# gcorso/disco-diffdock

Measured on AMD Instinct MI355X. Metric: complexes/sec, 20-step 40-sample inference, higher is better.
Workload: dtype f32

## Files before the change

disco_diffdock_amd/csrc/ddk_capi.hip:

```cpp
#include <math.h>
#include <algorithm>
#include <cmath>
#include <string.h>

#include "model.h"
#include "k_conv_common.h"

using namespace ddk;

namespace ddk {


int fail(ddk_ctx* ctx, int code, const std::string& msg) {
  if (ctx) ctx->err = msg;
  return code;
}

int hip_fail(ddk_ctx* ctx, hipError_t e, const char* what) {
  return fail(ctx, DDK_ERR_HIP, std::string(what) + ": " + hipGetErrorString(e));
}

hipError_t ctx_malloc(ddk_ctx* ctx, void** p, size_t bytes) {
  *p = nullptr;
  if (ctx->alloc_limit > 0 && ctx->dev_bytes + (int64_t)bytes > ctx->alloc_limit) { ctx->alloc_refusals++; return hipErrorOutOfMemory; }
// ... 306 lines not shown
  if (!bw || !bb || !bm || !bv) return DDK_ERR_INVALID;
  int ch = 0, f = 0;
  const int dims[4] = {1, 3, 3, 1};
  for (int b = 0; b < 4; ++b)
    for (int m = 0; m < out[b]; ++m, ++f) {
      const float sc = powf(bv->data[f] + 1e-5f, -0.5f) * bw->data[f];
      for (int d = 0; d < dims[b]; ++d, ++ch) {
        scale[ch] = sc;
        if (b == 0) { mean[ch] = bm->data[m]; bias[ch] = bb->data[m]; }
      }
    }
  return DDK_OK;
}

static int pack_x3(ddk_ctx* ctx, ConvLayerDev& L, int NG, const std::vector<float>& w1all, const std::vector<float>& w2all,
                   const std::vector<float>& b2all) {
  const size_t w1sz = 3 * 9 * 64 * 4, w2sz = (size_t)L.n_tiles * 9 * 64 * 4, b2sz = (size_t)L.n_tiles * 32;
  const int limbs = ctx->cfg.conv_kernel == 3 ? 3 : 2;
  const int tile_bytes = limbs == 3 ? W2X_TILE_BYTES : W2X2_TILE_BYTES, bias_off = limbs == 3 ? W2X_BIAS_OFF : W2X2_BIAS_OFF,
            desc_off = limbs == 3 ? W2X_DESC_OFF : W2X2_DESC_OFF, w1_tile_bytes = limbs == 3 ? W1X_TILE_BYTES : W1X2_TILE_BYTES;
  bool exact = true;
  auto split = [&exact, limbs](float v, uint16_t& hi, uint16_t& mid, uint16_t& lo) {
    const _Float16 h = (_Float16)v;
    const float r1 = v - (float)h;
    const _Float16 m = (_Float16)r1;
    const _Float16 l = (_Float16)(r1 - (float)m);
    memcpy(&hi, &h, 2); memcpy(&mid, &m, 2); memcpy(&lo, &l, 2);
    if (limbs == 3) {
      const double back = (double)(float)h + (double)(float)m + (double)(float)l;
      if (std::fabs(v) >= 0.5f ? back != (double)v : std::fabs(back - (double)v) > 0x1p-25) exact = false;
    } else {
      const double back = (double)(float)h + (double)(float)m;
      if (std::fabs(back - (double)v) > std::max(0x1p-22 * std::fabs((double)v), 0x1p-25)) exact = false;
    }
  };
  auto range_scale = [](const float* v, size_t n, const float* v2, size_t n2) {
    float m = 0.f;
    for (size_t i = 0; i < n; ++i) m = std::max(m, std::fabs(v[i]));
    for (size_t i = 0; i < n2; ++i) m = std::max(m, std::fabs(v2[i]));
    int e = 0;
    std::frexp(std::max(m, 0x1p-40f), &e);
    return std::ldexp(1.0f, 15 - e);
  };
  std::vector<uint8_t> w2x((size_t)(NG * L.n_tiles + 4) * tile_bytes, 0), w1x((size_t)NG * 3 * w1_tile_bytes, 0);
  auto frags = [&](const float* src, float sc, uint8_t* dst) {
    for (int r = 0; r < 36; ++r)
      for (int lane = 0; lane < 64; ++lane) {
        const float v = src[((size_t)(r / 4) * 64 + lane) * 4 + (r & 3)] * sc;
        const int s_ = r / 8, i = r % 8;
        const size_t off = s_ < 4 ? (size_t)s_ * 1024 + lane * 16 + 2 * i : (size_t)4096 + lane * 8 + 2 * i;
        uint16_t h, m, l;
        split(v, h, m, l);
        memcpy(dst + off, &h, 2); memcpy(dst + W2X_LIMB_BYTES + off, &m, 2);
        if (limbs == 3) memcpy(dst + 2 * W2X_LIMB_BYTES + off, &l, 2);
      }
  };
  for (int g = 0; g < NG; ++g) {
    const float* w2 = w2all.data() + g * w2sz;
    const float* w1 = w1all.data() + g * w1sz;
    const float* b2 = b2all.data() + g * b2sz;
    const float sc1 = range_scale(w1, w1sz, nullptr, 0), sc2 = range_scale(w2, w2sz, nullptr, 0);
    L.w1s[g] = sc1; L.w2s[g] = sc2;
    for (int t = 0; t < L.n_tiles; ++t) {
      uint8_t* rec = w2x.data() + ((size_t)g * L.n_tiles + t) * tile_bytes;
      frags(w2 + (size_t)t * 2304, sc2, rec);
      memcpy(rec + bias_off, b2 + (size_t)t * 32, 128);
      const int32_t dq[2] = {x_tile_word(L.h_tiles[t].w0), L.h_tiles[t].chan0};
      if (dq[0] < 0) return fail(ctx, DDK_ERR_INVALID, "internal: a vector tile of the conv layout does not sit on a T1O / T1E row quad");
      memcpy(rec + desc_off, dq, 8);
    }
    for (int T = 0; T < 3; ++T) frags(w1 + (size_t)T * 2304, sc1, w1x.data() + ((size_t)g * 3 + T) * w1_tile_bytes);
  }
  if (!exact)
    return fail(ctx, DDK_ERR_INVALID, limbs == 3 ? "internal: the three-limb fp16 split of a conv weight is not exact"
                                                 : "internal: the two-limb fp16 split of a conv weight leaves its 2^-22 window");
  L.h_w2x = w2x; L.h_w1x = w1x;
  L.epi_ok = conv_epilogue_shapes_ok(L.h_tiles);
  L.limbs = limbs;
  if (ctx->host_only) return DDK_OK;
  L.w2x = (uint8_t*)dev_alloc(ctx, w2x.size());
  L.w1x = (uint8_t*)dev_alloc(ctx, w1x.size());
  if (!L.w2x || !L.w1x) return fail(ctx, DDK_ERR_NOMEM, "device allocation failed while packing conv weights (f16 limbs)");
  if (hipMemcpy(L.w2x, w2x.data(), w2x.size(), hipMemcpyHostToDevice) != hipSuccess ||
      hipMemcpy(L.w1x, w1x.data(), w1x.size(), hipMemcpyHostToDevice) != hipSuccess)
    return fail(ctx, DDK_ERR_HIP, "f16-limb weight upload failed");
  return DDK_OK;
}

static int build_conv_layer(ddk_ctx* ctx, int mode, int l, ConvLayerDev& L) {
  const ddk_config& c = ctx->cfg;
  const int ns = c.ns;
  std::vector<int> rowmap;
  std::vector<float> rowscale;
  std::vector<TileDesc> tiles;
  int rc = build_layout(ctx, mode, l, L, rowmap, rowscale, tiles);
  if (rc) return rc;
  const int NG = mode == 0 ? 4 : 9;
// ... 69 lines not shown
  L.h_bn_bias.assign((size_t)n_bn * XW, 0.f);
  if (c.batch_norm)
    for (int g = 0; g < n_bn; ++g) {
      const std::string pre = "conv_layers." + std::to_string(mode == 0 ? l : 9 * l + g) + ".batch_norm";
      if ((rc = fold_batch_norm(ctx, pre, L.out_mul, L.h_bn_mean.data() + (size_t)g * XW, L.h_bn_scale.data() + (size_t)g * XW,
                                L.h_bn_bias.data() + (size_t)g * XW)))
        return rc;
    }
  L.h_w1p.resize(NG); L.h_b1p.resize(NG); L.h_w2p.resize(NG); L.h_b2p.resize(NG);
  for (int g = 0; g < NG; ++g) {
    L.h_w1p[g].assign(w1all.begin() + g * w1sz, w1all.begin() + (g + 1) * w1sz);
    L.h_b1p[g].assign(b1all.begin() + g * b1sz, b1all.begin() + (g + 1) * b1sz);
    L.h_w2p[g].assign(w2all.begin() + g * w2sz, w2all.begin() + (g + 1) * w2sz);
    L.h_b2p[g].assign(b2all.begin() + g * b2sz, b2all.begin() + (g + 1) * b2sz);
  }
  if (mode == 0 && c.conv_kernel != 1 && (rc = pack_x3(ctx, L, NG, w1all, w2all, b2all))) return rc;
  if (mode == 1 && c.conv_kernel != 1) {
    std::vector<int> rmx = rowmap;
    std::vector<float> rsx = rowscale;
    for (int t = 0; t + 1 < L.n_tiles; ++t) {
      if ((tiles[t].w0 & 3) != T_TV || (tiles[t].w0 >> 16) != F_T2E) continue;
      if ((tiles[t + 1].w0 & 3) != T_TV || (tiles[t + 1].w0 >> 16) != F_T2E + 12) return fail(ctx, DDK_ERR_INVALID, "internal: the two tiles of a T2E row group are not adjacent");
      for (int rq = 0; rq < 3; ++rq)
        for (int hh = 0; hh < 2; ++hh) {
          const size_t a = (size_t)t * 32 + 8 * rq + 4 * hh, b = (size_t)(t + 1) * 32 + 8 * rq + 4 * hh;
          if (rowmap[b + 2] >= 0 || rowmap[b + 3] >= 0) return fail(ctx, DDK_ERR_INVALID, "internal: a T2E row group holds more than six rows");
          for (int j = 0; j < 2; ++j) {
            rmx[a + j] = -1; rsx[a + j] = 0.f;
            rmx[a + 2 + j] = rowmap[a + j]; rsx[a + 2 + j] = rowscale[a + j];
            rmx[b + j] = rowmap[a + 2 + j]; rsx[b + j] = rowscale[a + 2 + j];
            rmx[b + 2 + j] = rowmap[b + j]; rsx[b + 2 + j] = rowscale[b + j];
// ... 363 lines not shown
    ConvLayerDev& L = head ? ctx->head[l - 100] : ctx->conv[l];
    if (g < 0 || g >= L.n_groups) return fail(ctx, DDK_ERR_INVALID, "bad export index");
    const std::string it(item);
    if (it == "w1p") { src = L.h_w1p[g].data(); n = L.h_w1p[g].size(); }
    else if (it == "b1p") { src = L.h_b1p[g].data(); n = L.h_b1p[g].size(); }
    else if (it == "w2p") { src = L.h_w2p[g].data(); n = L.h_w2p[g].size(); }
    else if (it == "b2p") { src = L.h_b2p[g].data(); n = L.h_b2p[g].size(); }
    else if (it == "wn") { src = L.h_wn.data(); n = L.h_wn.size(); }
    else if (it == "bnp") { src = L.h_bnp.data(); n = L.h_bnp.size(); }
    else if (it == "tiles") { src = L.h_tiles.data(); n = L.h_tiles.size() * (sizeof(TileDesc) / 4); }
    else if (it == "bn_mean") { src = L.h_bn_mean.data(); n = L.h_bn_mean.size(); }
    else if (it == "bn_scale") { src = L.h_bn_scale.data(); n = L.h_bn_scale.size(); }
    else if (it == "bn_bias") { src = L.h_bn_bias.data(); n = L.h_bn_bias.size(); }
    else if (it == "w1x") { src = L.h_w1x.data(); n = L.h_w1x.size() / 4; }
    else if (it == "w2x") { src = L.h_w2x.data(); n = L.h_w2x.size() / 4; }
    else if (it == "xscale") { static thread_local float sc[8]; for (int k = 0; k < 4; ++k) { sc[k] = L.w1s[k]; sc[4 + k] = L.w2s[k]; } src = sc; n = 8; }
    else return fail(ctx, DDK_ERR_INVALID, "unknown export item");
  } else {
    return fail(ctx, DDK_ERR_INVALID, "unknown export name");
  }
  if (buf) {
    if (cap_words < n) return fail(ctx, DDK_ERR_INVALID, "export buffer too small");
    memcpy(buf, src, (size_t)n * 4);
  }
  return n;
}

int ddk_debug_split3(ddk_ctx* ctx, const float* x, int64_t n, int32_t group, float* hi, float* mid, float* lo, float* scale, void* stream) {
  if (!ctx || ctx->host_only) return DDK_ERR_STATE;
  if (n < 0 || group < 1 || !x || !hi || !mid || !lo || !scale) return fail(ctx, DDK_ERR_INVALID, "ddk_debug_split3: bad argument");
// ... 6 lines not shown
```

disco_diffdock_amd/csrc/ddk_internal.h:

```cpp
#pragma once
#include <hip/hip_runtime.h>
#include <stdint.h>

#include <map>
#include <string>
#include <vector>

#include "../../include/ddk.h"
#include "../../include/ddk_debug.h"

namespace ddk {

constexpr int NS = 24;
constexpr int NV = 6;
constexpr int XW = 2 * NS + 6 * NV;
constexpr int NE = 3 * NS;
constexpr int OFF_P = NS;
constexpr int OFF_Q = NS + 3 * NV;
constexpr int OFF_C = NS + 6 * NV;

constexpr int F_A = 0;
constexpr int F_C = NS;
constexpr int F_T1O = 2 * NS;
constexpr int F_T1E = F_T1O + 6 * NV;
// ... 15 lines not shown
template <int MODE> struct ConvTraits;
template <> struct ConvTraits<0> { static constexpr int WAVES = CONV_WAVES, FS = F_STRIDE; };
template <> struct ConvTraits<1> { static constexpr int WAVES = 6, FS = F_STRIDE2; };
template <int MODE> constexpr size_t conv_lds_bytes() { return (size_t)(ConvTraits<MODE>::WAVES * 32 * ConvTraits<MODE>::FS + 2 * W2_TILE_FLOATS + 16) * 4; }
static_assert(conv_lds_bytes<1>() <= 160 * 1024, "LDS budget (l<=2)");
constexpr int CONV_MAX_GROUPS = 9;
constexpr int W2X_LIMB_BYTES = 4 * 1024 + 512;
constexpr int W2X_BIAS_OFF = 3 * W2X_LIMB_BYTES;
constexpr int W2X_DESC_OFF = W2X_BIAS_OFF + 128;
constexpr int W2X_TILE_BYTES = W2X_DESC_OFF + 16;
constexpr int W1X_TILE_BYTES = 3 * W2X_LIMB_BYTES;
constexpr int W2X2_BIAS_OFF = 2 * W2X_LIMB_BYTES;
constexpr int W2X2_DESC_OFF = W2X2_BIAS_OFF + 128;
constexpr int W2X2_TILE_BYTES = W2X2_DESC_OFF + 16;
constexpr int W1X2_TILE_BYTES = 2 * W2X_LIMB_BYTES;
constexpr int W1L_LIMB_BYTES = 1024 + 512;
constexpr int W1L_BYTES = 3 * 2 * W1L_LIMB_BYTES;
constexpr int CONV_TRACE_TILES = 1024;
constexpr int FX_A = 0, FX_C = NS, FX_R = 2 * NS, FX_PQ = FX_R + 6 * NV, FX_STRIDE = FX_PQ + 12 + 4;
static_assert(FX_STRIDE == 100 && FX_A == F_A && FX_C == F_C, "F row layout (three-limb f16)");
constexpr int W2X_STAGES = 4;
constexpr size_t CONV_X_LDS_BYTES = (size_t)CONV_WAVES * 32 * FX_STRIDE * 4 + W2X_STAGES * W2X_TILE_BYTES + 16;
static_assert(CONV_X_LDS_BYTES <= 160 * 1024 && W2X_TILE_BYTES % 16 == 0, "LDS budget (three-limb f16)");
constexpr size_t CONV_X2_LDS_BYTES = (size_t)CONV_WAVES * 32 * FX_STRIDE * 4 + W2X_STAGES * W2X2_TILE_BYTES + W1L_BYTES + 16;
static_assert(CONV_X2_LDS_BYTES <= 160 * 1024 && W2X2_TILE_BYTES % 16 == 0 && W1L_BYTES % 16 == 0, "LDS budget (two-limb f16)");

enum TileKind : int {
  T_RA = 0,
  T_RT = 1,
  T_TV = 2,
  T_RTS = 3
};
// ... 32 lines not shown
      if (first != odd) w0 |= 0x4000 << half;
    }
  }
  return (w0 & 0xffff) | (nf << 16);
}

struct ConvLayerDev {
  int n_tiles = 0;
  bool has_weights = false;
  int W = 0;
  int din = 0, dout = 0;
  float* w1p[4] = {};
  float* b1p[4] = {};
  float* w2r[4] = {};
  uint8_t* w1x = nullptr;
  uint8_t* w2x = nullptr;
  float w1s[CONV_MAX_GROUPS] = {1, 1, 1, 1, 1, 1, 1, 1, 1}, w2s[CONV_MAX_GROUPS] = {1, 1, 1, 1, 1, 1, 1, 1, 1};
  int limbs = 2;
  bool epi_ok = false;
  int n_cols = 0;
  int col_start[17] = {};
  float* wn = nullptr;
  float* bnp = nullptr;
  std::vector<float> h_wn, h_bnp;
  float* bn_mean = nullptr;
  float* bn_scale = nullptr;
  float* bn_bias = nullptr;
  std::vector<std::vector<float>> h_w1p, h_b1p, h_w2p, h_b2p;
  std::vector<float> h_bn_mean, h_bn_scale, h_bn_bias;
  int n_groups = 4;
  std::vector<TileDesc> h_tiles;
  std::vector<uint8_t> h_w1x, h_w2x;
  int n_in[4] = {}, n_out[4] = {}, blk_off[4] = {};
  int in_mul[4] = {}, out_mul[4] = {};
};

constexpr int PRE_W = 4 * NE;
static inline int pre_pos(int o) {
  const int r32 = o < 64 ? o % 32 : o - 64, hh = (r32 >> 2) & 1;
  return o < 64 ? hh * 36 + (o / 32) * 16 + (r32 & 3) + 4 * (r32 >> 3) : hh * 36 + 32 + (r32 & 3);
}

struct HostTensor {
  std::vector<int64_t> shape;
  std::vector<float> data;
};

// ... 116 lines not shown
```

disco_diffdock_amd/csrc/k_conv.hip:

```cpp
#include <stdlib.h>

#include "k_conv_common.h"
#include "k_node.h"
#include "model.h"

namespace ddk {

__device__ __forceinline__ void load_frags(float4 (&a)[9], f32x16& B, const float* w, const float* b) {
#pragma unroll
  for (int s4 = 0; s4 < 9; ++s4) a[s4] = ld4(w + s4 * 256);
#pragma unroll
  for (int j = 0; j < 4; ++j) {
    const float4 v = ld4(b + 4 * j);
    B[4 * j + 0] = v.x; B[4 * j + 1] = v.y; B[4 * j + 2] = v.z; B[4 * j + 3] = v.w;
  }
}

__device__ __forceinline__ f32x16 burst(const float4 (&a)[9], const float (&h)[36], const f32x16& C) {
  f32x16 D = MFMA(a[0].x, h[0], C);
  D = MFMA(a[0].y, h[1], D);
  D = MFMA(a[0].z, h[2], D);
  D = MFMA(a[0].w, h[3], D);
#pragma unroll
  for (int s4 = 1; s4 < 9; ++s4) {
// ... 486 lines not shown
  float* row = (A.sum_g2 != nullptr && g == 2) ? A.sum_g2 + (size_t)(s_last - A.g2_node_off) * XW
                                               : A.sum + ((size_t)s_last * A.n_slots + ((A.slots >> (2 * g)) & 3)) * XW;
  if (lane < dout) row[lane] = acc0;
  if (lane + 64 < dout) row[lane + 64] = acc1;
}

void conv_det_fix(const ConvKArgs& k, const ConvLaunch& a, int dout, hipStream_t s) {
  const int64_t tiles = a.edge_bound / 32 + 8 * CONV_MAX_GROUPS + (int64_t)CONV_WAVES * a.det_nr;
  hipLaunchKernelGGL(conv_det_fix_kernel, dim3((unsigned)((tiles + 3) / 4)), dim3(256), 0, s, k, dout);
}

hipError_t launch_conv_fused(const ConvLayerDev& L, const ConvLaunch& a, int n_cu, hipStream_t s) {
  if (L.w2x != nullptr && (a.mode == 0 || (a.mode == 1 && a.pre == nullptr)))
    return L.limbs == 2 ? launch_conv_fused_x2(L, a, n_cu, s) : launch_conv_fused_x(L, a, n_cu, s);
  ConvKArgs k;
  k.w1x = nullptr; k.w2x = nullptr;
  for (int g = 0; g < CONV_MAX_GROUPS; ++g) { k.w1s[g] = 1.0f; k.w1u[g] = 1.0f; k.w2s[g] = 1.0f; k.w2u[g] = 1.0f; }
  k.x = a.x; k.src = a.src; k.dst = a.dst; k.edge_attr = a.edge_attr; k.sh = a.sh; k.sum = a.sum;
  k.counter = a.counter;
  k.w1p = L.w1p[0]; k.b1p = L.b1p[0]; k.w2r = L.w2r[0]; k.n_tiles = L.n_tiles;
  k.n_cols = L.n_cols;
  for (int c = 0; c <= L.n_cols; ++c) k.col_start[c] = L.col_start[c];
  k.sum_g2 = a.sum_g2; k.g2_node_off = a.g2_node_off;
  k.n_groups = a.n_groups; k.n_active = a.n_active; k.n_slots = a.n_slots; k.slots = a.slots; k.wmap = a.wmap;
  if (a.gbeg) { k.gbeg = a.gbeg; k.gend = a.gend; }
  else { k.gbeg = a.tile_info + 5; k.gend = a.tile_info + 6; }
  k.pre = a.pre; k.part = a.part; k.det_rng = a.det_rng; k.det_nr = a.det_nr;
  if (a.part != nullptr) {
    if (a.mode != 0) return hipErrorInvalidValue;
    hipError_t e = (a.gather && a.pre != nullptr) ? launch_conv_t<true, 0, true, true>(k, n_cu, s)
                                                  : (!a.gather ? launch_conv_t<false, 0, false, true>(k, n_cu, s) : hipErrorInvalidValue);
// ... 47 lines not shown
```

disco_diffdock_amd/csrc/k_conv_common.h:

```cpp
#pragma once
#include "ddk_internal.h"

namespace ddk {

typedef float f32x16 __attribute__((ext_vector_type(16)));

struct ConvKArgs {
  const float* x;
  const int32_t* src;
  const int32_t* dst;
  const float* edge_attr;
  const float* sh;
  const float* pre;
  float* sum;
  int32_t* counter;
  const float* w1p;
  const float* b1p;
  const float* w2r;
  const uint8_t* w1x;
  const uint8_t* w2x;
  float w1s[CONV_MAX_GROUPS], w1u[CONV_MAX_GROUPS], w2s[CONV_MAX_GROUPS], w2u[CONV_MAX_GROUPS];
  int n_tiles;
  int n_cols;
  int col_start[17];
  float* part;
  float* sum_g2;
  int g2_node_off;
  int n_groups, n_active, n_slots;
  uint32_t slots;
  uint64_t wmap;
  const int32_t* gbeg;
  const int32_t* gend;
  const int32_t* det_rng = nullptr;
  int det_nr = 0;
// ... 133 lines not shown
```

disco_diffdock_amd/csrc/k_conv_x.hip:

```cpp
#include <stdlib.h>

#include "k_conv_common.h"

#ifdef X3_TWO_LIMBS
#define conv_x3_kernel conv_x2_kernel
#define launch_conv_fused_x launch_conv_fused_x2
#define conv_prepare_device_x conv_prepare_device_x2
#include "k_conv_x_epi2_gen.inc"
#define X3_TILE_BYTES W2X2_TILE_BYTES
#define X3_BIAS_OFF W2X2_BIAS_OFF
#define X3_DESC_OFF W2X2_DESC_OFF
#define X3_W1_TILE_BYTES W1X2_TILE_BYTES
#define X3_LDS_BYTES CONV_X2_LDS_BYTES
#define X3_W1L_BYTES W1L_BYTES
#define X3_TWO true
#define X3_SUM(r) D0[r]
#define X3_TAIL3(a_lh, a_hm) (void)(a_lh); D0 = MFMA16(a_hm, HT.mh, D0); D0 = MFMA16(a_hm, HT.hm, D0);
#define X3_STEP(MF, ah, am, al, bh, bm, bl)   \
  (void)(al);                                 \
  D0 = MF(ah, bm, D0);                        \
  D0 = MF(am, bh, D0);                        \
  D0 = MF(ah, bh, D0);
#define X3_FRAG(f, off) f.h = *reinterpret_cast<const f16x8*>(ringl + (off)); f.m = *reinterpret_cast<const f16x8*>(ringl + W2X_LIMB_BYTES + (off));
#define X3_TAIL_LO(SO) th
// ... 29 lines not shown
#define X3_RIDERS_3 X3_PAIR(0x100) X3_PAIR(0x100) X3_PAIR(0x100) X3_PAIR(0x100) X3_BARE X3_BARE
#define X3_TAIL_BARES X3_BARE X3_BARE X3_BARE
#endif

namespace ddk {

typedef _Float16 f16x8 __attribute__((ext_vector_type(8)));
typedef _Float16 f16x4 __attribute__((ext_vector_type(4)));
typedef unsigned int u32x4 __attribute__((vector_size(16)));
#define MFMA16(a, b, c) __builtin_amdgcn_mfma_f32_32x32x16_f16((a), (b), (c), 0, 0, 0)
#define MFMA8(a, b, c) __builtin_amdgcn_mfma_f32_32x32x8f16((a), (b), (c), 0, 0, 0)

struct W1Split { f16x8 h, m, l; f16x4 th, tm, tl; };
#ifdef X3_TWO_LIMBS
template <class TY> __device__ __forceinline__ TY w1_lo(const char*, const TY& hi) { return hi; }
__device__ __forceinline__ W1Split w1_split(const char* w1l, const char*, int T, int lane) {
  const char* wt = w1l + T * (2 * W1L_LIMB_BYTES);
  W1Split f;
  f.h = *reinterpret_cast<const f16x8*>(wt + lane * 16);
  f.m = *reinterpret_cast<const f16x8*>(wt + W1L_LIMB_BYTES + lane * 16);
  f.th = *reinterpret_cast<const f16x4*>(wt + 1024 + lane * 8);
  f.tm = *reinterpret_cast<const f16x4*>(wt + W1L_LIMB_BYTES + 1024 + lane * 8);
  f.l = f.h; f.tl = f.th;
  return f;
}
#else
template <class TY> __device__ __forceinline__ TY w1_lo(const char* p, const TY&) { return *reinterpret_cast<const TY*>(p); }
__device__ __forceinline__ W1Split w1_split(const char*, const char* w1, int T, int lane) {
  const char* wt = w1 + (size_t)T * W1X_TILE_BYTES;
  W1Split f;
  f.h = *reinterpret_cast<const f16x8*>(wt + lane * 16);
  f.m = *reinterpret_cast<const f16x8*>(wt + W2X_LIMB_BYTES + lane * 16);
  f.l = *reinterpret_cast<const f16x8*>(wt + 2 * W2X_LIMB_BYTES + lane * 16);
  f.th = *reinterpret_cast<const f16x4*>(wt + 1024 + lane * 16);
  f.tm = *reinterpret_cast<const f16x4*>(wt + W2X_LIMB_BYTES + 1024 + lane * 16);
  f.tl = *reinterpret_cast<const f16x4*>(wt + 2 * W2X_LIMB_BYTES + 1024 + lane * 16);
  return f;
}
#endif

__device__ __forceinline__ float range_scale(float m, float& inv) {
  const uint32_t eb = max((__float_as_uint(m) >> 23) & 0xffu, 87u);
  inv = __uint_as_float((eb - 14u) << 23);
// ... 264 lines not shown
      const float4 r4 = *reinterpret_cast<const float4*>(wr2 + fo0);
      if (has1_s) { if (has1) {
        const float4 r1 = *reinterpret_cast<const float4*>(wr0 + fo1);
        const float4 r3 = *reinterpret_cast<const float4*>(wr1 + fo1);
        const float4 r5 = *reinterpret_cast<const float4*>(wr2 + fo1);
        *reinterpret_cast<float4*>(ring + fo1) = r1;
        *reinterpret_cast<float4*>(ring + X3_TILE_BYTES + fo1) = r3;
        *reinterpret_cast<float4*>(ring + 2 * X3_TILE_BYTES + fo1) = r5;
      } }
      *reinterpret_cast<float4*>(ring + fo0) = r0;
      *reinterpret_cast<float4*>(ring + X3_TILE_BYTES + fo0) = r2;
      *reinterpret_cast<float4*>(ring + 2 * X3_TILE_BYTES + fo0) = r4;
    }
#ifdef X3_TWO_LIMBS
    if constexpr (SPLIT) {
      const int gw_s = __builtin_amdgcn_readfirstlane(gw);
      if (gw_s != gw_lds) {
        if (wave < 6) {
          const char* wsrc = reinterpret_cast<const char*>(A.w1x) + ((size_t)gw_s * 3 + (wave >> 1)) * X3_W1_TILE_BYTES + (wave & 1) * W2X_LIMB_BYTES;
          const float4 c16 = *reinterpret_cast<const float4*>(wsrc + lane * 16);
          const float2 c8 = *reinterpret_cast<const float2*>(wsrc + 1024 + lane * 16);
          *reinterpret_cast<float4*>(w1l + wave * W1L_LIMB_BYTES + lane * 16) = c16;
          *reinterpret_cast<float2*>(w1l + wave * W1L_LIMB_BYTES + 1024 + lane * 8) = c8;
        }
        gw_lds = gw_s;
        lds_barrier();
      }
    }
#endif

    const SegF seg = make_segf(make_segctl(sn, el, nvalid, valid));
    stamp(5);

    const float4 shv = ld4(A.sh + (size_t)e * 4);
    float4 mainv[NS / 4];
    float2 pv2[3 * NV / 2];
    {
      const float* xr = A.x + (size_t)dn * XW;
#pragma unroll
      for (int j = 0; j < NS / 4; ++j) mainv[j] = ld4(xr + (hh ? OFF_C : 0) + 4 * j);
#pragma unroll
      for (int j = 0; j < 3 * NV / 2; ++j) pv2[j] = ld2(xr + (hh ? OFF_Q : OFF_P) + 2 * j);
    }

    Limbs H;
    TailB HT;
    float osc, bsc2;
    {
      float h[36];
      const char* w1 = reinterpret_cast<const char*>(A.w1x) + (size_t)gw * 3 * X3_W1_TILE_BYTES;
      (void)w1;
      if constexpr (SPLIT) {
        float4 psv[9], pdv[9];
        {
          const float* ps = A.pre + ((size_t)sn * 4 + (gw & 1)) * NE + 36 * hh;
          const float* pd = A.pre + ((size_t)dn * 4 + 2 + (gw >> 1)) * NE + 36 * hh;
#pragma unroll
          for (int j = 0; j < 9; ++j) { psv[j] = ld4(ps + 4 * j); pdv[j] = ld4(pd + 4 * j); }
        }
        float bin[12];
        {
          const float* pe = A.edge_attr + (size_t)e * NS + 12 * hh;
#pragma unroll
          for (int j = 0; j < 3; ++j) {
            const float4 a = ld4(pe + 4 * j);
            bin[4 * j + 0] = a.x; bin[4 * j + 1] = a.y; bin[4 * j + 2] = a.z; bin[4 * j + 3] = a.w;
          }
// ... 15 lines not shown
        const float bsc = s1 * A.w1s[gw], usc = inv1 * A.w1u[gw];
#pragma unroll
        for (int T = 0; T < 3; ++T) {
          f32x16 D0, D1;
#pragma unroll
          for (int j = 0; j < 4; ++j) {
            if (T < 2 || j == 0) {
              const float4 u = psv[4 * T + j], w = pdv[4 * T + j];
              D0[4 * j + 0] = (u.x + w.x) * bsc; D0[4 * j + 1] = (u.y + w.y) * bsc; D0[4 * j + 2] = (u.z + w.z) * bsc; D0[4 * j + 3] = (u.w + w.w) * bsc;
            } else {
              D0[4 * j + 0] = 0.0f; D0[4 * j + 1] = 0.0f; D0[4 * j + 2] = 0.0f; D0[4 * j + 3] = 0.0f;
            }
          }
#pragma unroll
          for (int r = 0; r < 16; ++r) D1[r] = 0.0f;
          const W1Split wf = w1_split(w1l, w1, T, lane);
          X3_STEP(MFMA16, wf.h, wf.m, wf.l, b0h, b0m, b0l)
          {
            const f16x4 ah = wf.th, am = wf.tm, al = wf.tl;
            const f16x8 a_hm = __builtin_shufflevector(ah, am, 0, 1, 2, 3, 4, 5, 6, 7), a_lh = __builtin_shufflevector(al, ah, 0, 1, 2, 3, 4, 5, 6, 7);
            D0 = MFMA16(a_hm, b1_mh, D0);
#ifndef X3_TWO_LIMBS
            D1 = MFMA16(a_lh, b1_hl, D1);
#else
            (void)a_lh; (void)b1_hl;
#endif
            D0 = MFMA16(a_hm, b1_hm, D0);
          }
          const int nr = T < 2 ? 16 : 4;
#pragma unroll
          for (int r = 0; r < 16; ++r)
            if (r < nr) h[16 * T + r] = fmaxf(X3_SUM(r), 0.0f) * usc;
        }
      } else {
        float bin[36];
        {
          const float *pe, *pxs, *pxd;
          if (GATHER) {
            pe = A.edge_attr + (size_t)e * NS + 12 * hh;
            pxs = A.x + (size_t)sn * XW + 12 * hh;
            pxd = A.x + (size_t)dn * XW + 12 * hh;
          } else {
            pe = A.edge_attr + (size_t)e * NE + 12 * hh;
            pxs = pe + NS;
            pxd = pe + 2 * NS;
          }
#pragma unroll
          for (int j = 0; j < 3; ++j) {
// ... 49 lines not shown
      for (int j = 0; j < 36; ++j) m2 = fmaxf(m2, h[j]);
      m2 = fmaxf(m2, __shfl_xor(m2, 32));
      float inv2;
      const float s2 = range_scale(m2, inv2);
      stamp(6);
      make_limbs(H, h, s2);
      HT = make_tailb(H);
      bsc2 = s2 * A.w2s[gw];
      osc = inv2 * A.w2u[gw];
    }

    const float s0 = shv.x, vx = shv.y, vy = shv.z, vz = shv.w;
    {
      const int o_main_dst = hh ? FX_C : FX_A, r0 = hh ? NV : 0;
#pragma unroll
      for (int j = 0; j < NS / 4; ++j) *reinterpret_cast<float4*>(Fr + o_main_dst + 4 * j) = mainv[j];
      float pv[3 * NV];
#pragma unroll
      for (int j = 0; j < 3 * NV / 2; ++j) { pv[2 * j] = pv2[j].x; pv[2 * j + 1] = pv2[j].y; }
#pragma unroll
      for (int m = 0; m < NV; ++m) {
        const float px = pv[3 * m], py = pv[3 * m + 1], pz = pv[3 * m + 2];
        Fr[FX_PQ + (m < 4 ? 4 * hh + m : 8 + 2 * hh + (m - 4))] = (px * vx + py * vy + pz * vz) * inv_s3;
        const int r = r0 + m;
        float* Pr = Fr + FX_R + 12 * (r >> 2) + (r & 3);
        Pr[0] = px;
        Pr[4] = py;
        Pr[8] = pz;
      }
    }
    stamp(7);
// ... 263 lines not shown
    e = hipFuncSetAttribute(reinterpret_cast<const void*>(&conv_x3_kernel<true, true, false, true>), hipFuncAttributeMaxDynamicSharedMemorySize,
                            (int)X3_LDS_BYTES);
  if (e == hipSuccess)
    e = hipFuncSetAttribute(reinterpret_cast<const void*>(&conv_x3_kernel<true, false, false, false, 1>), hipFuncAttributeMaxDynamicSharedMemorySize,
                            (int)X3_LDS_BYTES);
  if (e == hipSuccess)
    e = hipFuncSetAttribute(reinterpret_cast<const void*>(&conv_x3_kernel<false, false, false, false, 1>), hipFuncAttributeMaxDynamicSharedMemorySize,
                            (int)X3_LDS_BYTES);
  return e;
}

void conv_det_fix(const ConvKArgs& k, const ConvLaunch& a, int dout, hipStream_t s);

hipError_t launch_conv_fused_x(const ConvLayerDev& L, const ConvLaunch& a, int n_cu, hipStream_t s) {
  if (a.mode != 0 && a.mode != 1) return hipErrorInvalidValue;
  ConvXArgs X;
  ConvKArgs& k = X.k;
  k.x = a.x; k.src = a.src; k.dst = a.dst; k.edge_attr = a.edge_attr; k.sh = a.sh; k.sum = a.sum;
  k.counter = a.counter;
  k.w1p = nullptr; k.b1p = L.b1p[0]; k.w2r = nullptr; k.w1x = L.w1x; k.w2x = L.w2x; k.n_tiles = L.n_tiles;
  for (int g = 0; g < CONV_MAX_GROUPS; ++g) { k.w1s[g] = L.w1s[g]; k.w1u[g] = 1.0f / L.w1s[g]; k.w2s[g] = L.w2s[g]; k.w2u[g] = 1.0f / L.w2s[g]; }
  k.n_cols = L.n_cols;
  for (int c = 0; c <= L.n_cols; ++c) k.col_start[c] = L.col_start[c];
  k.sum_g2 = a.sum_g2; k.g2_node_off = a.g2_node_off;
  k.n_groups = a.n_groups; k.n_active = a.n_active; k.n_slots = a.n_slots; k.slots = a.slots; k.wmap = a.wmap;
  if (a.gbeg) { k.gbeg = a.gbeg; k.gend = a.gend; }
  else { k.gbeg = a.tile_info + 5; k.gend = a.tile_info + 6; }
  k.pre = a.pre; k.part = a.part; k.det_rng = a.det_rng; k.det_nr = a.det_nr;
  X.trace = nullptr; X.trace_coarse = a.trace_coarse;
  if (a.mode == 1) {
    if (a.pre != nullptr || a.part != nullptr || a.trace != nullptr) return hipErrorInvalidValue;
    if (a.gather) hipLaunchKernelGGL((conv_x3_kernel<true, false, false, false, 1>), dim3(n_cu), dim3(64 * CONV_WAVES), X3_LDS_BYTES, s, X);
    else hipLaunchKernelGGL((conv_x3_kernel<false, false, false, false, 1>), dim3(n_cu), dim3(64 * CONV_WAVES), X3_LDS_BYTES, s, X);
    return hipGetLastError();
  }
// ... 20 lines not shown
```

disco_diffdock_amd/csrc/model.hip:

```cpp
#include <math.h>
#include <string.h>

#include <algorithm>
#include <thread>

#include "k_philox.h"
#include "model.h"

namespace ddk {

std::vector<float> cols(const HostTensor* t, int c0, int c1) {
  const int rows = (int)t->shape[0], nc = (int)t->shape[1];
  std::vector<float> o((size_t)rows * (c1 - c0));
  for (int r = 0; r < rows; ++r)
    for (int c = c0; c < c1; ++c) o[(size_t)r * (c1 - c0) + (c - c0)] = t->data[(size_t)r * nc + c];
  return o;
}

static bool smearing(ddk_ctx* ctx, const char* name, float stop, EdgeMlpDev& m, std::vector<float>* host_off, float* host_coeff) {
  std::vector<float> off(DE);
  auto it = ctx->weights.find(std::string(name) + "_distance_expansion.offset");
  if (it != ctx->weights.end() && it->second.data.size() == (size_t)DE) off = it->second.data;
  else for (int k = 0; k < DE; ++k) off[k] = stop * (float)k / (float)(DE - 1);
  const double d = (double)(off[1] - off[0]);
// ... 437 lines not shown
  F.e_src = cx->e_src; F.e_dst = cx->e_dst; F.e_aux = cx->e_aux; F.info = cx->info; F.e_emb = cx->e_emb; F.e_sh = cx->e_sh;
  F.lig = M->dev.lig_edge; F.rec = M->dev.rec_edge; F.cross = M->dev.cross_edge; F.sp = sp;
  F.n_lig_total = B * n_lig; F.n_rec = n_rec; F.n_shared = dedup ? cx->E_rr : 0;
  F.g2_live_only = (dedup && prune && c.num_conv_layers == 5) ? 1 : 0;
  F.patch_off = (dedup && patched) ? cx->patch_off : -1;
  F.latent_dim = c.latent_dim; F.lig_latent = cx->lig_latent; F.rec_latent = cx->rec_latent; F.unconditional = cx->unconditional;
  const int64_t cap_b = (int64_t)B * ((int64_t)cx->M + (int64_t)n_lig * LIG_CAP + 2LL * n_lig * n_rec + cx->E_rr) + cx->E_rr;
  const int64_t feat_cap = (cap_b < cx->edge_cap ? cap_b : cx->edge_cap) + (F.patch_off >= 0 ? (int64_t)B * cx->E_rr + 256 : 0);
  float* xin = cx->xa;
  float* xout = cx->xb;
  NodeEmbedArgs NE_;
  NE_.lig_static = cx->lig_node_static; NE_.rec_static = cx->rec_node_static; NE_.sp = sp; NE_.B = B; NE_.n_lig = n_lig; NE_.n_rec = n_rec;
  NE_.x = xin; NE_.lig_latent = cx->lig_latent; NE_.rec_latent = cx->rec_latent; NE_.lig_w_lat = M->dev.lig_w_lat; NE_.rec_w_lat = M->dev.rec_w_lat;
  NE_.lig_unc = M->dev.lig_node_unc; NE_.rec_unc = M->dev.rec_node_unc; NE_.unconditional = cx->unconditional; NE_.latent_dim = c.latent_dim;
  const bool split = ctx->conv[0].wn != nullptr && cx->pre != nullptr;
  if (split) {
    NodePreArgs PA = {};
    PA.x_out = xin; PA.n_lig_total = B * n_lig; PA.n_rec_total = B * n_rec; PA.n_rec = n_rec;
    PA.wn = ctx->conv[0].wn; PA.bnp = ctx->conv[0].bnp; PA.pre = cx->pre; PA.n_slots = 1; PA.lig_roles = 15; PA.rec_roles = 15;
    CK(launch_edge_features_node(F, feat_cap, PA, NE_, s), "edge features + node embed + node_pre");
  } else {
    CK(launch_edge_features(F, feat_cap, s), "edge features");
    CK(launch_node_embed(NE_, s), "node embed");
  }
  if (!cx->sum_clean) {
    CK(hipMemsetAsync(cx->sum, 0, (size_t)cx->max_batch * (n_lig + n_rec) * XW * sizeof(float) * (c.deterministic ? 2 : 1), s), "memset sum");
    CK(hipMemsetAsync(cx->sum_rr0, 0, (size_t)n_rec * XW * sizeof(float), s), "memset sum_rr0");
  }
  cx->sum_clean = false;
  bool rr0_dirty = false;
  const int NL = c.num_conv_layers;
  int32_t* prof_slot = nullptr;
  if (ctx->prof && ctx->prof_slots + 1 <= ctx->prof_cap) prof_slot = ctx->prof_edges + (size_t)PROF_INTS * ctx->prof_slots;
  for (int l = 0; l < NL; ++l) {
// ... 37 lines not shown
    if (ctx->conv_trace != nullptr && ctx->conv_trace_layer == l) { a.trace = ctx->conv_trace; a.trace_coarse = ctx->conv_trace_coarse; }
    CK(launch_conv_fused(L, a, ctx->n_cu, s), "conv_fused");
    if (prof_slot) {
      CK(hipEventRecord(pr.b, s), "event record");
      ctx->prof_recs.push_back(pr);
    }
    const bool clear_rr0 = rr0_dirty && !shared0;
    if (split && l + 1 < NL) {
      NodePreArgs PA = {};
      PA.sum = cx->sum; PA.deg = cx->deg; PA.x_in = xin; PA.bn_mean = L.bn_mean; PA.bn_scale = L.bn_scale; PA.bn_bias = L.bn_bias;
      PA.dout = L.dout; PA.x_out = xout; PA.sum_rr0 = shared0 ? cx->sum_rr0 : nullptr; PA.n_lig_total = B * n_lig; PA.n_rec_total = B * n_rec;
      PA.rr0_mask = (shared0 && patched) ? cx->rr_mask : nullptr;
      PA.n_rec = n_rec; PA.zero_extra = clear_rr0 ? cx->sum_rr0 : nullptr; PA.n_extra = clear_rr0 ? (int64_t)n_rec * XW : 0;
      PA.wn = ctx->conv[l + 1].wn; PA.bnp = ctx->conv[l + 1].bnp; PA.pre = cx->pre; PA.n_slots = c.deterministic ? 2 : 1;
      const bool next_lig_only = (l + 1 == NL - 1) && !cx->keep_rec;
      PA.lig_roles = next_lig_only ? 0x7 : 0xF; PA.rec_roles = next_lig_only ? 0x4 : 0xF;
      PA.levels = prune ? cx->levels : nullptr; PA.max_level = l == NL - 2 ? 0 : (l == NL - 3 ? 1 : (l == NL - 4 ? 2 : 3));
      CK(launch_node_finalize_pre(PA, true, s), "node_finalize_pre");
    } else
    CK(launch_node_finalize(cx->sum, cx->deg, xin, L.bn_mean, L.bn_scale, L.bn_bias, lig_only ? (int64_t)B * n_lig : N, L.dout, XW, xout, s,
                            shared0 ? cx->sum_rr0 : nullptr, (int64_t)B * n_lig, n_rec, 1, clear_rr0 ? cx->sum_rr0 : nullptr,
                            clear_rr0 ? (int64_t)n_rec * XW : 0, c.deterministic ? 2 : 1, (shared0 && patched) ? cx->rr_mask : nullptr), "node_finalize");
    if (clear_rr0) rr0_dirty = false;
    float* t = xin; xin = xout; xout = t;
  }
  cx->x_last = xin;
  cx->last_B = B;
  cx->last_full = cx->keep_rec;
  cx->sum_clean = !rr0_dirty;
  if (M->confidence_mode) return DDK_OK;
  const bool torsion = !c.no_torsion && tor_out != nullptr && cx->R > 0;
// ... 817 lines not shown
```

Measured before the change: 49.51.

## Fold sender-node features into edge GEMM1 instead of per-node precompute

In the two-limb split conv path, the sender (destination-node) contribution to the first edge MLP layer is no longer precomputed per node. Instead it is computed inside the edge GEMM by extending the MFMA K dimension to 48, combining edge attributes with sender scalar features. A new packed weight buffer (w1sx) holds the reordered rows, and the LDS copy is resized to match. Node pre-kernels now only compute the receiver roles, with a reduced role mask. This trades per-node precompute work and its memory traffic for extra MFMA work and on-the-fly fp16 limb splitting per edge.

After: 51.38, median of 6. 3.8% higher.

```diff
diff --git a/disco_diffdock_amd/csrc/ddk_capi.hip b/disco_diffdock_amd/csrc/ddk_capi.hip
--- a/disco_diffdock_amd/csrc/ddk_capi.hip
+++ b/disco_diffdock_amd/csrc/ddk_capi.hip
@@ -344,7 +344,7 @@
 }
 
 static int pack_x3(ddk_ctx* ctx, ConvLayerDev& L, int NG, const std::vector<float>& w1all, const std::vector<float>& w2all,
-                   const std::vector<float>& b2all) {
+                   const std::vector<float>& b2all, bool sender_k48 = false) {
   const size_t w1sz = 3 * 9 * 64 * 4, w2sz = (size_t)L.n_tiles * 9 * 64 * 4, b2sz = (size_t)L.n_tiles * 32;
   const int limbs = ctx->cfg.conv_kernel == 3 ? 3 : 2;
   const int tile_bytes = limbs == 3 ? W2X_TILE_BYTES : W2X2_TILE_BYTES, bias_off = limbs == 3 ? W2X_BIAS_OFF : W2X2_BIAS_OFF,
@@ -372,7 +372,7 @@
     std::frexp(std::max(m, 0x1p-40f), &e);
     return std::ldexp(1.0f, 15 - e);
   };
-  std::vector<uint8_t> w2x((size_t)(NG * L.n_tiles + 4) * tile_bytes, 0), w1x((size_t)NG * 3 * w1_tile_bytes, 0);
+  std::vector<uint8_t> w2x((size_t)(NG * L.n_tiles + 4) * tile_bytes, 0), w1x((size_t)NG * 3 * w1_tile_bytes, 0), w1sx(limbs == 2 && sender_k48 ? (size_t)NG * W1L_BYTES : 0, 0);
   auto frags = [&](const float* src, float sc, uint8_t* dst) {
     for (int r = 0; r < 36; ++r)
       for (int lane = 0; lane < 64; ++lane) {
@@ -400,17 +400,31 @@
       memcpy(rec + desc_off, dq, 8);
     }
     for (int T = 0; T < 3; ++T) frags(w1 + (size_t)T * 2304, sc1, w1x.data() + ((size_t)g * 3 + T) * w1_tile_bytes);
+    if (!w1sx.empty())
+      for (int T = 0; T < 3; ++T)
+        for (int r = 0; r < 24; ++r)
+          for (int lane = 0; lane < 64; ++lane) {
+            const int r72 = w1s_k72_register(r);
+            const float v = w1[(size_t)T * 2304 + ((size_t)(r72 / 4) * 64 + lane) * 4 + (r72 & 3)] * sc1;
+            uint8_t* dst = w1sx.data() + (size_t)g * W1L_BYTES + (size_t)T * 2 * W1L_LIMB_BYTES + (size_t)(r / 8) * 1024 + lane * 16 + 2 * (r % 8);
+            uint16_t h, m, l;
+            split(v, h, m, l);
+            memcpy(dst, &h, 2); memcpy(dst + W1L_LIMB_BYTES, &m, 2);
+          }
   }
   if (!exact)
     return fail(ctx, DDK_ERR_INVALID, limbs == 3 ? "internal: the three-limb fp16 split of a conv weight is not exact"
                                                  : "internal: the two-limb fp16 split of a conv weight leaves its 2^-22 window");
-  L.h_w2x = w2x; L.h_w1x = w1x;
+  L.h_w2x = w2x; L.h_w1x = w1x; L.h_w1sx = w1sx;
+  L.sender_in_gemm1 = !w1sx.empty();
   L.epi_ok = conv_epilogue_shapes_ok(L.h_tiles);
   L.limbs = limbs;
   if (ctx->host_only) return DDK_OK;
   L.w2x = (uint8_t*)dev_alloc(ctx, w2x.size());
   L.w1x = (uint8_t*)dev_alloc(ctx, w1x.size());
-  if (!L.w2x || !L.w1x) return fail(ctx, DDK_ERR_NOMEM, "device allocation failed while packing conv weights (f16 limbs)");
+  if (!w1sx.empty()) L.w1sx = (uint8_t*)dev_alloc(ctx, w1sx.size());
+  if (!L.w2x || !L.w1x || (!w1sx.empty() && !L.w1sx)) return fail(ctx, DDK_ERR_NOMEM, "device allocation failed while packing conv weights (f16 limbs)");
+  if (!w1sx.empty() && hipMemcpy(L.w1sx, w1sx.data(), w1sx.size(), hipMemcpyHostToDevice) != hipSuccess) return fail(ctx, DDK_ERR_HIP, "f16-limb weight upload failed");
   if (hipMemcpy(L.w2x, w2x.data(), w2x.size(), hipMemcpyHostToDevice) != hipSuccess ||
       hipMemcpy(L.w1x, w1x.data(), w1x.size(), hipMemcpyHostToDevice) != hipSuccess)
     return fail(ctx, DDK_ERR_HIP, "f16-limb weight upload failed");
@@ -510,7 +524,7 @@
     L.h_w2p[g].assign(w2all.begin() + g * w2sz, w2all.begin() + (g + 1) * w2sz);
     L.h_b2p[g].assign(b2all.begin() + g * b2sz, b2all.begin() + (g + 1) * b2sz);
   }
-  if (mode == 0 && c.conv_kernel != 1 && (rc = pack_x3(ctx, L, NG, w1all, w2all, b2all))) return rc;
+  if (mode == 0 && c.conv_kernel != 1 && (rc = pack_x3(ctx, L, NG, w1all, w2all, b2all, true))) return rc;
   if (mode == 1 && c.conv_kernel != 1) {
     std::vector<int> rmx = rowmap;
     std::vector<float> rsx = rowscale;
@@ -904,6 +918,7 @@
     else if (it == "bn_bias") { src = L.h_bn_bias.data(); n = L.h_bn_bias.size(); }
     else if (it == "w1x") { src = L.h_w1x.data(); n = L.h_w1x.size() / 4; }
     else if (it == "w2x") { src = L.h_w2x.data(); n = L.h_w2x.size() / 4; }
+    else if (it == "w1sx") { src = L.h_w1sx.data(); n = L.h_w1sx.size() / 4; }
     else if (it == "xscale") { static thread_local float sc[8]; for (int k = 0; k < 4; ++k) { sc[k] = L.w1s[k]; sc[4 + k] = L.w2s[k]; } src = sc; n = 8; }
     else return fail(ctx, DDK_ERR_INVALID, "unknown export item");
   } else {
diff --git a/disco_diffdock_amd/csrc/ddk_internal.h b/disco_diffdock_amd/csrc/ddk_internal.h
--- a/disco_diffdock_amd/csrc/ddk_internal.h
+++ b/disco_diffdock_amd/csrc/ddk_internal.h
@@ -53,8 +53,9 @@
 constexpr int W2X2_DESC_OFF = W2X2_BIAS_OFF + 128;
 constexpr int W2X2_TILE_BYTES = W2X2_DESC_OFF + 16;
 constexpr int W1X2_TILE_BYTES = 2 * W2X_LIMB_BYTES;
-constexpr int W1L_LIMB_BYTES = 1024 + 512;
+constexpr int W1L_LIMB_BYTES = 3 * 1024;
 constexpr int W1L_BYTES = 3 * 2 * W1L_LIMB_BYTES;
+static inline int w1s_k72_register(int r) { return r < 12 ? r : r + 12; }
 constexpr int CONV_TRACE_TILES = 1024;
 constexpr int FX_A = 0, FX_C = NS, FX_R = 2 * NS, FX_PQ = FX_R + 6 * NV, FX_STRIDE = FX_PQ + 12 + 4;
 static_assert(FX_STRIDE == 100 && FX_A == F_A && FX_C == F_C, "F row layout (three-limb f16)");
@@ -117,9 +118,11 @@
   float* b1p[4] = {};
   float* w2r[4] = {};
   uint8_t* w1x = nullptr;
+  uint8_t* w1sx = nullptr;
   uint8_t* w2x = nullptr;
   float w1s[CONV_MAX_GROUPS] = {1, 1, 1, 1, 1, 1, 1, 1, 1}, w2s[CONV_MAX_GROUPS] = {1, 1, 1, 1, 1, 1, 1, 1, 1};
   int limbs = 2;
+  bool sender_in_gemm1 = false;
   bool epi_ok = false;
   int n_cols = 0;
   int col_start[17] = {};
@@ -133,7 +136,7 @@
   std::vector<float> h_bn_mean, h_bn_scale, h_bn_bias;
   int n_groups = 4;
   std::vector<TileDesc> h_tiles;
-  std::vector<uint8_t> h_w1x, h_w2x;
+  std::vector<uint8_t> h_w1x, h_w2x, h_w1sx;
   int n_in[4] = {}, n_out[4] = {}, blk_off[4] = {};
   int in_mul[4] = {}, out_mul[4] = {};
 };
diff --git a/disco_diffdock_amd/csrc/k_conv.hip b/disco_diffdock_amd/csrc/k_conv.hip
--- a/disco_diffdock_amd/csrc/k_conv.hip
+++ b/disco_diffdock_amd/csrc/k_conv.hip
@@ -524,7 +524,7 @@
   if (L.w2x != nullptr && (a.mode == 0 || (a.mode == 1 && a.pre == nullptr)))
     return L.limbs == 2 ? launch_conv_fused_x2(L, a, n_cu, s) : launch_conv_fused_x(L, a, n_cu, s);
   ConvKArgs k;
-  k.w1x = nullptr; k.w2x = nullptr;
+  k.w1x = nullptr; k.w1sx = nullptr; k.w2x = nullptr;
   for (int g = 0; g < CONV_MAX_GROUPS; ++g) { k.w1s[g] = 1.0f; k.w1u[g] = 1.0f; k.w2s[g] = 1.0f; k.w2u[g] = 1.0f; }
   k.x = a.x; k.src = a.src; k.dst = a.dst; k.edge_attr = a.edge_attr; k.sh = a.sh; k.sum = a.sum;
   k.counter = a.counter;
diff --git a/disco_diffdock_amd/csrc/k_conv_common.h b/disco_diffdock_amd/csrc/k_conv_common.h
--- a/disco_diffdock_amd/csrc/k_conv_common.h
+++ b/disco_diffdock_amd/csrc/k_conv_common.h
@@ -18,6 +18,7 @@
   const float* b1p;
   const float* w2r;
   const uint8_t* w1x;
+  const uint8_t* w1sx;
   const uint8_t* w2x;
   float w1s[CONV_MAX_GROUPS], w1u[CONV_MAX_GROUPS], w2s[CONV_MAX_GROUPS], w2u[CONV_MAX_GROUPS];
   int n_tiles;
diff --git a/disco_diffdock_amd/csrc/k_conv_x.hip b/disco_diffdock_amd/csrc/k_conv_x.hip
--- a/disco_diffdock_amd/csrc/k_conv_x.hip
+++ b/disco_diffdock_amd/csrc/k_conv_x.hip
@@ -67,19 +67,9 @@
 struct W1Split { f16x8 h, m, l; f16x4 th, tm, tl; };
 #ifdef X3_TWO_LIMBS
 template <class TY> __device__ __forceinline__ TY w1_lo(const char*, const TY& hi) { return hi; }
-__device__ __forceinline__ W1Split w1_split(const char* w1l, const char*, int T, int lane) {
-  const char* wt = w1l + T * (2 * W1L_LIMB_BYTES);
-  W1Split f;
-  f.h = *reinterpret_cast<const f16x8*>(wt + lane * 16);
-  f.m = *reinterpret_cast<const f16x8*>(wt + W1L_LIMB_BYTES + lane * 16);
-  f.th = *reinterpret_cast<const f16x4*>(wt + 1024 + lane * 8);
-  f.tm = *reinterpret_cast<const f16x4*>(wt + W1L_LIMB_BYTES + 1024 + lane * 8);
-  f.l = f.h; f.tl = f.th;
-  return f;
-}
 #else
 template <class TY> __device__ __forceinline__ TY w1_lo(const char* p, const TY&) { return *reinterpret_cast<const TY*>(p); }
-__device__ __forceinline__ W1Split w1_split(const char*, const char* w1, int T, int lane) {
+__device__ __forceinline__ W1Split w1_split(const char* w1, int T, int lane) {
   const char* wt = w1 + (size_t)T * W1X_TILE_BYTES;
   W1Split f;
   f.h = *reinterpret_cast<const f16x8*>(wt + lane * 16);
@@ -374,15 +364,18 @@
     }
 #ifdef X3_TWO_LIMBS
     if constexpr (SPLIT) {
+      static_assert(W1L_BYTES / 16 == 2 * 64 * CONV_WAVES + 128, "the copy below moves 1152 chunks");
       const int gw_s = __builtin_amdgcn_readfirstlane(gw);
       if (gw_s != gw_lds) {
-        if (wave < 6) {
-          const char* wsrc = reinterpret_cast<const char*>(A.w1x) + ((size_t)gw_s * 3 + (wave >> 1)) * X3_W1_TILE_BYTES + (wave & 1) * W2X_LIMB_BYTES;
-          const float4 c16 = *reinterpret_cast<const float4*>(wsrc + lane * 16);
-          const float2 c8 = *reinterpret_cast<const float2*>(wsrc + 1024 + lane * 16);
-          *reinterpret_cast<float4*>(w1l + wave * W1L_LIMB_BYTES + lane * 16) = c16;
-          *reinterpret_cast<float2*>(w1l + wave * W1L_LIMB_BYTES + 1024 + lane * 8) = c8;
-        }
+        const char* wsrc = reinterpret_cast<const char*>(A.w1sx) + (size_t)gw_s * W1L_BYTES;
+        const float4 c0 = *reinterpret_cast<const float4*>(wsrc + 16 * tid);
+        const float4 c1 = *reinterpret_cast<const float4*>(wsrc + 16 * (tid + 64 * WAVES));
+        if (wave < 2) {
+          const float4 c2 = *reinterpret_cast<const float4*>(wsrc + 16 * (tid + 128 * WAVES));
+          *reinterpret_cast<float4*>(w1l + 16 * (tid + 128 * WAVES)) = c2;
+        }
+        *reinterpret_cast<float4*>(w1l + 16 * tid) = c0;
+        *reinterpret_cast<float4*>(w1l + 16 * (tid + 64 * WAVES)) = c1;
         gw_lds = gw_s;
         lds_barrier();
       }
@@ -392,11 +385,13 @@
     const SegF seg = make_segf(make_segctl(sn, el, nvalid, valid));
     stamp(5);
 
-    const float4 shv = ld4(A.sh + (size_t)e * 4);
+    constexpr bool SENDK = SPLIT && X3_TWO;
+    float4 shv;
     float4 mainv[NS / 4];
     float2 pv2[3 * NV / 2];
-    {
-      const float* xr = A.x + (size_t)dn * XW;
+    const float* xr = A.x + (size_t)dn * XW;
+    if constexpr (!SENDK) {
+      shv = ld4(A.sh + (size_t)e * 4);
 #pragma unroll
       for (int j = 0; j < NS / 4; ++j) mainv[j] = ld4(xr + (hh ? OFF_C : 0) + 4 * j);
 #pragma unroll
@@ -411,6 +406,67 @@
       const char* w1 = reinterpret_cast<const char*>(A.w1x) + (size_t)gw * 3 * X3_W1_TILE_BYTES;
       (void)w1;
       if constexpr (SPLIT) {
+#ifdef X3_TWO_LIMBS
+        float4 psv[9];
+        {
+          const float* ps = A.pre + ((size_t)sn * 4 + (gw & 1)) * NE + 36 * hh;
+#pragma unroll
+          for (int j = 0; j < 9; ++j) psv[j] = ld4(ps + 4 * j);
+        }
+        float bin[24];
+        {
+          const float* pe = A.edge_attr + (size_t)e * NS + 12 * hh;
+#pragma unroll
+          for (int j = 0; j < 3; ++j) {
+            const float4 a = ld4(pe + 4 * j);
+            bin[4 * j + 0] = a.x; bin[4 * j + 1] = a.y; bin[4 * j + 2] = a.z; bin[4 * j + 3] = a.w;
+          }
+#pragma unroll
+          for (int j = 0; j < 3; ++j) mainv[j] = ld4(xr + 12 * hh + 4 * j);
+        }
+        shv = ld4(A.sh + (size_t)e * 4);
+#pragma unroll
+        for (int j = 0; j < 3; ++j) mainv[3 + j] = ld4(xr + OFF_C + 12 * hh + 4 * j);
+#pragma unroll
+        for (int j = 0; j < 3 * NV / 2; ++j) pv2[j] = ld2(xr + (hh ? OFF_Q : OFF_P) + 2 * j);
+#pragma unroll
+        for (int j = 0; j < 3; ++j) { bin[12 + 4 * j + 0] = mainv[j].x; bin[12 + 4 * j + 1] = mainv[j].y; bin[12 + 4 * j + 2] = mainv[j].z; bin[12 + 4 * j + 3] = mainv[j].w; }
+        float m1 = 0.0f;
+#pragma unroll
+        for (int j = 0; j < 24; ++j) m1 = fmaxf(m1, fabsf(bin[j]));
+        m1 = fmaxf(m1, __shfl_xor(m1, 32));
+        float inv1;
+        const float s1 = range_scale(m1, inv1);
+        f16x8 bh[3], bm[3];
+#pragma unroll
+        for (int k = 0; k < 3; ++k)
+#pragma unroll
+          for (int i = 0; i < 8; ++i) { const Limb3 q = split3(bin[8 * k + i] * s1); bh[k][i] = q.h; bm[k][i] = q.m; }
+        const float bsc = s1 * A.w1s[gw], usc = inv1 * A.w1u[gw];
+#pragma unroll
+        for (int T = 0; T < 3; ++T) {
+          f32x16 D0;
+#pragma unroll
+          for (int j = 0; j < 4; ++j) {
+            if (T < 2 || j == 0) {
+              const float4 u = psv[4 * T + j];
+              D0[4 * j + 0] = u.x * bsc; D0[4 * j + 1] = u.y * bsc; D0[4 * j + 2] = u.z * bsc; D0[4 * j + 3] = u.w * bsc;
+            } else {
+              D0[4 * j + 0] = 0.0f; D0[4 * j + 1] = 0.0f; D0[4 * j + 2] = 0.0f; D0[4 * j + 3] = 0.0f;
+            }
+          }
+          const char* wt = w1l + T * (2 * W1L_LIMB_BYTES) + lane * 16;
+#pragma unroll
+          for (int k = 0; k < 3; ++k) {
+            const f16x8 ah = *reinterpret_cast<const f16x8*>(wt + k * 1024), am = *reinterpret_cast<const f16x8*>(wt + W1L_LIMB_BYTES + k * 1024);
+            X3_STEP(MFMA16, ah, am, ah, bh[k], bm[k], bh[k])
+          }
+          const int nr = T < 2 ? 16 : 4;
+#pragma unroll
+          for (int r = 0; r < 16; ++r)
+            if (r < nr) h[16 * T + r] = fmaxf(D0[r], 0.0f) * usc;
+        }
+#else
         float4 psv[9], pdv[9];
         {
           const float* ps = A.pre + ((size_t)sn * 4 + (gw & 1)) * NE + 36 * hh;
@@ -456,17 +512,13 @@
           }
 #pragma unroll
           for (int r = 0; r < 16; ++r) D1[r] = 0.0f;
-          const W1Split wf = w1_split(w1l, w1, T, lane);
+          const W1Split wf = w1_split(w1, T, lane);
           X3_STEP(MFMA16, wf.h, wf.m, wf.l, b0h, b0m, b0l)
           {
             const f16x4 ah = wf.th, am = wf.tm, al = wf.tl;
             const f16x8 a_hm = __builtin_shufflevector(ah, am, 0, 1, 2, 3, 4, 5, 6, 7), a_lh = __builtin_shufflevector(al, ah, 0, 1, 2, 3, 4, 5, 6, 7);
             D0 = MFMA16(a_hm, b1_mh, D0);
-#ifndef X3_TWO_LIMBS
             D1 = MFMA16(a_lh, b1_hl, D1);
-#else
-            (void)a_lh; (void)b1_hl;
-#endif
             D0 = MFMA16(a_hm, b1_hm, D0);
           }
           const int nr = T < 2 ? 16 : 4;
@@ -474,6 +526,7 @@
           for (int r = 0; r < 16; ++r)
             if (r < nr) h[16 * T + r] = fmaxf(X3_SUM(r), 0.0f) * usc;
         }
+#endif
       } else {
         float bin[36];
         {
@@ -553,7 +606,10 @@
     {
       const int o_main_dst = hh ? FX_C : FX_A, r0 = hh ? NV : 0;
 #pragma unroll
-      for (int j = 0; j < NS / 4; ++j) *reinterpret_cast<float4*>(Fr + o_main_dst + 4 * j) = mainv[j];
+      for (int j = 0; j < NS / 4; ++j) {
+        if constexpr (SENDK) *reinterpret_cast<float4*>(Fr + (j < 3 ? FX_A : FX_C - 12) + 12 * hh + 4 * j) = mainv[j];
+        else *reinterpret_cast<float4*>(Fr + o_main_dst + 4 * j) = mainv[j];
+      }
       float pv[3 * NV];
 #pragma unroll
       for (int j = 0; j < 3 * NV / 2; ++j) { pv[2 * j] = pv2[j].x; pv[2 * j + 1] = pv2[j].y; }
@@ -847,11 +903,12 @@
 
 hipError_t launch_conv_fused_x(const ConvLayerDev& L, const ConvLaunch& a, int n_cu, hipStream_t s) {
   if (a.mode != 0 && a.mode != 1) return hipErrorInvalidValue;
+  if (X3_TWO && a.gather && a.pre != nullptr && (!L.sender_in_gemm1 || L.w1sx == nullptr)) return hipErrorInvalidValue;
   ConvXArgs X;
   ConvKArgs& k = X.k;
   k.x = a.x; k.src = a.src; k.dst = a.dst; k.edge_attr = a.edge_attr; k.sh = a.sh; k.sum = a.sum;
   k.counter = a.counter;
-  k.w1p = nullptr; k.b1p = L.b1p[0]; k.w2r = nullptr; k.w1x = L.w1x; k.w2x = L.w2x; k.n_tiles = L.n_tiles;
+  k.w1p = nullptr; k.b1p = L.b1p[0]; k.w2r = nullptr; k.w1x = L.w1x; k.w1sx = L.w1sx; k.w2x = L.w2x; k.n_tiles = L.n_tiles;
   for (int g = 0; g < CONV_MAX_GROUPS; ++g) { k.w1s[g] = L.w1s[g]; k.w1u[g] = 1.0f / L.w1s[g]; k.w2s[g] = L.w2s[g]; k.w2u[g] = 1.0f / L.w2s[g]; }
   k.n_cols = L.n_cols;
   for (int c = 0; c <= L.n_cols; ++c) k.col_start[c] = L.col_start[c];
diff --git a/disco_diffdock_amd/csrc/model.hip b/disco_diffdock_amd/csrc/model.hip
--- a/disco_diffdock_amd/csrc/model.hip
+++ b/disco_diffdock_amd/csrc/model.hip
@@ -475,10 +475,12 @@
   NE_.x = xin; NE_.lig_latent = cx->lig_latent; NE_.rec_latent = cx->rec_latent; NE_.lig_w_lat = M->dev.lig_w_lat; NE_.rec_w_lat = M->dev.rec_w_lat;
   NE_.lig_unc = M->dev.lig_node_unc; NE_.rec_unc = M->dev.rec_node_unc; NE_.unconditional = cx->unconditional; NE_.latent_dim = c.latent_dim;
   const bool split = ctx->conv[0].wn != nullptr && cx->pre != nullptr;
+  const bool recv_only = split && ctx->conv[0].sender_in_gemm1;
+  const int role_mask = recv_only ? 0x3 : 0xF;
   if (split) {
     NodePreArgs PA = {};
     PA.x_out = xin; PA.n_lig_total = B * n_lig; PA.n_rec_total = B * n_rec; PA.n_rec = n_rec;
-    PA.wn = ctx->conv[0].wn; PA.bnp = ctx->conv[0].bnp; PA.pre = cx->pre; PA.n_slots = 1; PA.lig_roles = 15; PA.rec_roles = 15;
+    PA.wn = ctx->conv[0].wn; PA.bnp = ctx->conv[0].bnp; PA.pre = cx->pre; PA.n_slots = 1; PA.lig_roles = role_mask; PA.rec_roles = role_mask;
     CK(launch_edge_features_node(F, feat_cap, PA, NE_, s), "edge features + node embed + node_pre");
   } else {
     CK(launch_edge_features(F, feat_cap, s), "edge features");
@@ -546,7 +548,7 @@
       PA.n_rec = n_rec; PA.zero_extra = clear_rr0 ? cx->sum_rr0 : nullptr; PA.n_extra = clear_rr0 ? (int64_t)n_rec * XW : 0;
       PA.wn = ctx->conv[l + 1].wn; PA.bnp = ctx->conv[l + 1].bnp; PA.pre = cx->pre; PA.n_slots = c.deterministic ? 2 : 1;
       const bool next_lig_only = (l + 1 == NL - 1) && !cx->keep_rec;
-      PA.lig_roles = next_lig_only ? 0x7 : 0xF; PA.rec_roles = next_lig_only ? 0x4 : 0xF;
+      PA.lig_roles = (next_lig_only ? 0x7 : 0xF) & role_mask; PA.rec_roles = (next_lig_only ? 0x4 : 0xF) & role_mask;
       PA.levels = prune ? cx->levels : nullptr; PA.max_level = l == NL - 2 ? 0 : (l == NL - 3 ? 1 : (l == NL - 4 ? 2 : 3));
       CK(launch_node_finalize_pre(PA, true, s), "node_finalize_pre");
     } else
```
